# CEED/Laghos

Measured on AMD Instinct MI355X. Metric: Mdofs×steps/s on 3D Sedov -pa (Q3/Q2), higher is better.
Workload: dtype f64; 1 GPU; 3D Sedov -p 1 -m cube01_hex -rs 4 -ok 3 -ot 2 -pa (32^3 elements, E0/2^dim = 0.125); transport=none (one rank), elements=32768, h1_dofs=2738019, l2_dofs=884736, quad_points_per_element=216, rk_stages_executed=1300, ode=RK4, parallelism=elements1x1x1, zones_per_gpu=32x32x32

## Files before the change

include/laghos_hip.h:

```cpp
#ifndef LAGHOS_HIP_H
#define LAGHOS_HIP_H

#ifdef __cplusplus
extern "C" {
#endif

#define LGH_OK 0
#define LGH_ERR_ARG 1
#define LGH_ERR_UNSUPPORTED 2
#define LGH_ERR_HIP 3
#define LGH_ERR_COMM 4

#define LGH_SPACE_H1 0
#define LGH_SPACE_L2 1

typedef struct lgh_ctx lgh_ctx;

typedef struct lgh_config
{
   int dim, NE;
   int D1D, Q1D, L1D;
   int N;
   const int *h1_map;
   const double *B_h1;
// ... 20 lines not shown
void *lgh_stream(lgh_ctx *ctx);

double *lgh_qdata_stressJinvT(lgh_ctx *ctx);
double *lgh_qdata_Jac0inv(lgh_ctx *ctx);
double *lgh_qdata_rho0DetJ0w(lgh_ctx *ctx);
double *lgh_mass_D(lgh_ctx *ctx);
int lgh_mass_data_form(lgh_ctx *ctx, int *form);
int lgh_jac0inv_form(lgh_ctx *ctx, int *compact);
int lgh_mass_data_changed(lgh_ctx *ctx);
double *lgh_mass_diag(lgh_ctx *ctx);
int lgh_set_h0(lgh_ctx *ctx, double h0);
int lgh_get_h0(lgh_ctx *ctx, double *h0);
int lgh_set_dt_est(lgh_ctx *ctx, double dt_est);
int lgh_get_dt_est(lgh_ctx *ctx, double *dt_est);

int lgh_setup_rho0detj0(lgh_ctx *ctx, const double *x0, const double *rho0_l2,
                        const double *rho0_q, double *volume);

int lgh_force_mult(lgh_ctx *ctx, const double *x_l2, double *y_h1);
int lgh_force_mult_transpose(lgh_ctx *ctx, const double *v_h1, double *y_l2);

int lgh_mass_set_essential_tdofs(lgh_ctx *ctx, int comp);
int lgh_mass_eliminate_rhs(lgh_ctx *ctx, double *b);
int lgh_mass_mult(lgh_ctx *ctx, int space, const double *x, double *y);
int lgh_mass_mult_full(lgh_ctx *ctx, int space, const double *x, double *y);

int lgh_cg_solve(lgh_ctx *ctx, int space, const double *b, double *x, double rel_tol,
                 int max_iter, int *iters);
int lgh_l2_mass_solve_local(lgh_ctx *ctx, const double *b, double *x);

int lgh_qupdate(lgh_ctx *ctx, const double *S);
int lgh_qupdate_set_tiny_grad(lgh_ctx *ctx, double tiny_grad);
int lgh_qupdate_discard(lgh_ctx *ctx, int *mode, double *C_F);
int lgh_set_fused_forces(lgh_ctx *ctx, int on);
int lgh_qupdate_store_stress(lgh_ctx *ctx, int on);
int lgh_qupdate_stores_stress(lgh_ctx *ctx, int *on);
int lgh_qupdate_form(lgh_ctx *ctx, int *form);
int lgh_reset_quadrature_data(lgh_ctx *ctx);
int lgh_fused_force_mult(lgh_ctx *ctx, double *y_h1);
int lgh_fused_force_mult_transpose(lgh_ctx *ctx, double *y_l2);
int lgh_fused_force_e(lgh_ctx *ctx, double *y_e);
int lgh_quadrature_generation(lgh_ctx *ctx, unsigned long *gen, int *f1_valid, int *ftv_valid);
int lgh_get_fused_forces(lgh_ctx *ctx, int *f1, int *ftv);

int lgh_solve_velocity(lgh_ctx *ctx, const double *S, double *dS_dt, const double *one_l2,
                       double *rhs_h1, double *work_B, double rel_tol, int max_iter,
                       int *h1_iters);
int lgh_solve_energy(lgh_ctx *ctx, const double *S, const double *v_h1, double *dS_dt,
                     double *e_rhs, const double *e_source, double rel_tol, int max_iter,
                     int *l2_iters);
int lgh_solve_energy_begin(lgh_ctx *ctx, const double *S, const double *v_h1, double *dS_dt,
                           double *e_rhs, const double *e_source, double rel_tol, int max_iter);
int lgh_solve_energy_end(lgh_ctx *ctx, int *l2_iters);
int lgh_energy_lockstep_stats(lgh_ctx *ctx, long out[4]);

int lgh_vec_set(lgh_ctx *ctx, double *y, double a, long n);
int lgh_vec_copy(lgh_ctx *ctx, double *y, const double *x, long n);
int lgh_vec_axpby_pair(lgh_ctx *ctx, double *z1, double a1, const double *x1, double b1, double *z2, double a2, const double *x2, double b2,
                       const double *y, long n);
int lgh_vec_axpby(lgh_ctx *ctx, double *z, double a, const double *x, double b,
                  const double *y, long n);
int lgh_vec_dot(lgh_ctx *ctx, const double *x, const double *y, long n, double *result);
int lgh_vec_fingerprint(lgh_ctx *ctx, const double *x, long n, unsigned long long offset, unsigned long long out[2]);
int lgh_vec_fingerprint_shape(lgh_ctx *ctx, const double *x, long n, long out[4]);
int lgh_fingerprint_host(const void *words, long n, unsigned long long offset, unsigned long long out[2]);

// ... 106 lines not shown
```

laghos_amd/_lib.py:

```python
import ctypes
import os

_HERE = os.path.dirname(os.path.abspath(__file__))
LIB_PATH = os.path.join(_HERE, "liblaghos_hip.so")

c_dp = ctypes.c_void_p
c_int_p = ctypes.POINTER(ctypes.c_int)
c_dbl_p = ctypes.POINTER(ctypes.c_double)


class LghConfig(ctypes.Structure):
    _fields_ = [
        ("dim", ctypes.c_int), ("NE", ctypes.c_int),
        ("D1D", ctypes.c_int), ("Q1D", ctypes.c_int), ("L1D", ctypes.c_int),
        ("N", ctypes.c_int),
        ("h1_map", c_int_p),
        ("B_h1", c_dbl_p), ("G_h1", c_dbl_p), ("B_l2", c_dbl_p),
        ("weights", c_dbl_p), ("gamma", c_dbl_p),
        ("ess_count", ctypes.c_int * 3),
        ("ess", c_int_p * 3),
        ("owner", c_dbl_p),
        ("use_viscosity", ctypes.c_int), ("use_vorticity", ctypes.c_int),
        ("cfl", ctypes.c_double),
        ("order_v", ctypes.c_int),
# ... 49 lines not shown
    "lgh_vec_fingerprint_shape": (_I, [_P, _P, _L, ctypes.POINTER(ctypes.c_long)]),
    "lgh_fingerprint_host": (_I, [_P, _L, ctypes.c_ulonglong, ctypes.POINTER(ctypes.c_ulonglong)]),
    "lgh_internal_energy": (_I, [_P, _P, c_dbl_p]),
    "lgh_kinetic_energy": (_I, [_P, _P, c_dbl_p]),
    "lgh_sedov_setup": (_I, [_I, _D, _D, _D, _D, c_dbl_p]),
    "lgh_sedov_shock": (_I, [c_dbl_p, _D, c_dbl_p]),
    "lgh_sedov_eval_point": (_I, [c_dbl_p, _D, _D, c_dbl_p, c_dbl_p, c_dbl_p]),
    "lgh_sedov_eval": (_I, [_P, c_dbl_p, _D, _L, _P, _P, _P, _P]),
    "lgh_compute_density": (_I, [_P, _P, _P]),
    "lgh_sedov_density_error": (_I, [_P, _P, _P, c_dbl_p, _D, c_dbl_p, _I, c_dbl_p, c_dbl_p, c_dbl_p, c_dbl_p, c_dbl_p]),
    "lgh_sample_fields": (_I, [_P, _P, _P, _I, c_dbl_p, c_dbl_p, _P, _P, _P, _P, _P]),
    "lgh_sample_derived": (_I, [_P, _P, _I, c_dbl_p, c_dbl_p, c_dbl_p, _P, _P, _P, _P, _P]),
    "lgh_diagnostics_zones": (_I, [_P, _P, _P]),
    "lgh_diagnostics": (_I, [_P, _P, c_dbl_p]),
    "lgh_profile": (_I, [_P, _P, ctypes.POINTER(LghProfileSpec), c_dbl_p, ctypes.POINTER(ctypes.c_long)]),
    "lgh_get_timers": (_I, [_P, c_dbl_p, ctypes.POINTER(ctypes.c_long)]),
    "lgh_reset_timers": (_I, [_P]),
    "lgh_enable_timers": (_I, [_P, _I]),
    "lgh_ktime_begin": (_I, [_P, _I, _I]),
    "lgh_ktime_end": (_I, [_P, c_int_p, c_dbl_p]),
    "lgh_table_symmetry": (_I, [_P, c_int_p, c_int_p]),
    "lgh_k1_form": (_I, [_P, c_int_p]),
    "lgh_l2_mass_form": (_I, [_P, c_int_p, c_int_p]),
    "lgh_vcg_layout_stats": (_I, [_P, ctypes.POINTER(ctypes.c_long)]),
    "lgh_energy_lockstep_stats": (_I, [_P, ctypes.POINTER(ctypes.c_long)]),
    "lgh_mesh_order": (_I, [_P, ctypes.POINTER(ctypes.c_long)]),
    "lgh_mesh_order_host": (_I, [_I, _I, _I, _I, c_int_p, c_int_p, c_int_p, ctypes.POINTER(ctypes.c_long)]),
    "lgh_mass_data_form": (_I, [_P, c_int_p]),
    "lgh_jac0inv_form": (_I, [_P, c_int_p]),
    "lgh_mass_data_changed": (_I, [_P]),
    "lgh_comm_stats": (_I, [_P, c_int_p, ctypes.POINTER(ctypes.c_long), ctypes.POINTER(ctypes.c_long), c_int_p, c_int_p]),
    "lgh_qupdate_set_tiny_grad": (_I, [_P, _D]),
    "lgh_qupdate_discard": (_I, [_P, c_int_p, c_dbl_p]),
    "lgh_set_fused_forces": (_I, [_P, _I]),
    "lgh_qupdate_store_stress": (_I, [_P, _I]),
    "lgh_qupdate_stores_stress": (_I, [_P, c_int_p]),
    "lgh_qupdate_form": (_I, [_P, c_int_p]),
    "lgh_reset_quadrature_data": (_I, [_P]),
    "lgh_fused_force_mult": (_I, [_P, _P]),
    "lgh_fused_force_mult_transpose": (_I, [_P, _P]),
    "lgh_fused_force_e": (_I, [_P, _P]),
    "lgh_quadrature_generation": (_I, [_P, ctypes.POINTER(ctypes.c_ulong), c_int_p, c_int_p]),
    "lgh_get_fused_forces": (_I, [_P, c_int_p, c_int_p]),
    "lgh_comm_unique_id": (_I, [ctypes.c_char_p]),
    "lgh_comm_unique_id_shm": (_I, [ctypes.c_char_p]),
    "lgh_comm_init": (_I, [_P, _I, _I, ctypes.c_char_p]),
    "lgh_comm_set_neighbors": (_I, [_P, _I, c_int_p, c_int_p, ctypes.POINTER(c_int_p)]),
    "lgh_groups_to_neighbors": (_I, [_I, _I, _I, c_int_p, c_int_p, c_int_p, c_int_p, c_int_p, c_dbl_p, c_int_p, c_int_p,
                                     c_int_p, _I, c_int_p, _L]),
    "lgh_halo_sum": (_I, [_P, _P, _I]),
    "lgh_allreduce": (_I, [_P, c_dbl_p, _I]),
    "lgh_force_mult_E": (_I, [_P, _P, _P, _P]),
    "lgh_force_mult_transpose_E": (_I, [_P, _P, _P, _P]),
    "lgh_mass_apply_E": (_I, [_P, _I, _P, _P]),
    "lgh_test_vcg_k1": (_I, [_P, _P, _P, c_dbl_p, c_dbl_p, _I, _P, c_dbl_p]),
    "lgh_test_vcg_merged_faces": (_I, [_P, _P, ctypes.POINTER(ctypes.c_long)]),
    "lgh_test_vcg_k2": (_I, [_P, _I, _P, _P, _P, _P, c_dbl_p, c_dbl_p, c_dbl_p, c_dbl_p, c_dbl_p, ctypes.POINTER(ctypes.c_int)]),
    "lgh_test_exact_sum": (_I, [_P, _I, _L, _I, _I, c_dbl_p, c_dbl_p, ctypes.POINTER(ctypes.c_longlong),
                                ctypes.POINTER(ctypes.c_longlong), c_dbl_p, c_int_p]),
    "lgh_test_set_rank": (_I, [_P, _I, _I]),
    "lgh_test_word_peers": (_I, [_P, _I, ctypes.POINTER(ctypes.c_long)]),
    "lgh_test_halo_pack": (_I, [_P, _P, _I, _P]),
    "lgh_test_halo_combine": (_I, [_P, _P, _P, _I]),
    "lgh_test_rccl_self_sendrecv": (_I, [_P, _I, c_dbl_p]),
    "lgh_test_eig": (_I, [_P, _I, _I, _P, _P, _P]),
    "lgh_test_singular": (_I, [_P, _I, _I, _P, _P]),
# ... 38 lines not shown
```

laghos_amd/context.py:

```python
import ctypes

import numpy as np
import torch

from . import _lib
from ._lib import LghConfig, check


def _np_i32(a):
    return np.ascontiguousarray(a, dtype=np.int32)


def _np_f64(a):
    return np.ascontiguousarray(a, dtype=np.float64)


def _ptr(t):
    assert t.is_cuda and t.dtype == torch.float64 and t.is_contiguous()
    return ctypes.c_void_p(t.data_ptr())


def _dbl(a):
    assert isinstance(a, np.ndarray) and a.dtype == np.float64 and a.flags.c_contiguous
    return a.ctypes.data_as(_lib.c_dbl_p)
# ... 195 lines not shown

    def force_mult_transpose(self, v_h1, y_l2):
        check(self.lib.lgh_force_mult_transpose(self.h, _ptr(v_h1), _ptr(y_l2)))

    def mass_set_ess(self, comp):
        check(self.lib.lgh_mass_set_essential_tdofs(self.h, comp))

    def mass_eliminate_rhs(self, b):
        check(self.lib.lgh_mass_eliminate_rhs(self.h, _ptr(b)))

    def mass_mult(self, space, x, y, full=False):
        fn = self.lib.lgh_mass_mult_full if full else self.lib.lgh_mass_mult
        check(fn(self.h, space, _ptr(x), _ptr(y)))

    def cg_solve(self, space, b, x, rel_tol, max_iter):
        it = ctypes.c_int(0)
        check(self.lib.lgh_cg_solve(self.h, space, _ptr(b), _ptr(x), rel_tol, max_iter, ctypes.byref(it)))
        return it.value

    def l2_mass_solve_local(self, b, x):
        check(self.lib.lgh_l2_mass_solve_local(self.h, _ptr(b), _ptr(x)))

    def qupdate(self, S):
        check(self.lib.lgh_qupdate(self.h, _ptr(S)))

    def qupdate_set_tiny_grad(self, v):
        check(self.lib.lgh_qupdate_set_tiny_grad(self.h, float(v)))

    def qupdate_discard(self):
        m, cf = ctypes.c_int(-1), ctypes.c_double(0.0)
        check(self.lib.lgh_qupdate_discard(self.h, ctypes.byref(m), ctypes.byref(cf)))
        return m.value, cf.value

    def table_symmetry(self):
        a, b = ctypes.c_int(-1), ctypes.c_int(-1)
        check(self.lib.lgh_table_symmetry(self.h, ctypes.byref(a), ctypes.byref(b)))
        return a.value, b.value

    def k1_form(self):
        f = ctypes.c_int(-2)
        check(self.lib.lgh_k1_form(self.h, ctypes.byref(f)))
        return {0: "column", 2: "plane", 4: "slab", 5: "kron"}.get(f.value)

    def mesh_order(self):
        o = (ctypes.c_long * 8)()
        check(self.lib.lgh_mesh_order(self.h, o))
        return dict(structured=bool(o[0]), identity=bool(o[1]), components=int(o[2]), extent=(int(o[3]), int(o[4]), int(o[5])))

    def test_vcg_k1(self, r, d_old, rz, rz_prev, first):
        y = self.empty(3 * self.NE * self.ND)
        rz, rzp, den = _np_f64(rz), _np_f64(rz_prev), np.zeros(3)
        check(self.lib.lgh_test_vcg_k1(self.h, _ptr(r), _ptr(d_old) if d_old is not None else None, _dbl(rz), _dbl(rzp),
                                       int(bool(first)), _ptr(y), _dbl(den)))
        return y.view(3, -1), den

    def test_vcg_merged_faces(self):
        mask = np.zeros(self.NE * self.ND, dtype=np.uint8)
        n = ctypes.c_long(0)
        check(self.lib.lgh_test_vcg_merged_faces(self.h, mask.ctypes.data_as(ctypes.c_void_p), ctypes.byref(n)))
        return mask, n.value

    def test_vcg_k2(self, it, y_E, r, d, x, den, rz, rz_prev, alpha_prev):
        den, rz, rzp, al, out = _np_f64(den), _np_f64(rz), _np_f64(rz_prev), _np_f64(alpha_prev), np.zeros(3)
        form = ctypes.c_int(-1)
        check(self.lib.lgh_test_vcg_k2(self.h, int(it), _ptr(y_E), _ptr(r), _ptr(d), _ptr(x), _dbl(den), _dbl(rz), _dbl(rzp),
                                       _dbl(al), _dbl(out), ctypes.byref(form)))
# ... 264 lines not shown
```

laghos_amd/csrc/lgh_api.hip:

```cpp
#include <cstdarg>
#include <cstdlib>
#include <cmath>
#include <algorithm>
#include <limits>

#include "lgh_common.hpp"

#include <atomic>
#include <chrono>
#include <dlfcn.h>

namespace lgh
{

static thread_local char g_err[512] = "";
void set_error(const char *fmt, ...)
{
   va_list ap;
   va_start(ap, fmt);
   vsnprintf(g_err, sizeof(g_err), fmt, ap);
   va_end(ap);
}

__global__ void __launch_bounds__(256) vec_set_k(double *y, double a, long n)
// ... 245 lines not shown
   s.slab_exact = env_flag("LGH_SLAB_EXACT", 1);
   s.slab_merge = env_flag("LGH_SLAB_MERGE", 1);
   s.slab_defer = env_flag("LGH_SLAB_DEFER", 1);
   s.slab_ye_wide = env_flag("LGH_SLAB_YE_WIDE", 0);
   s.slab_dyn = env_flag("LGH_SLAB_DYN", -1);
   s.rz_limbs = env_flag("LGH_RZ_LIMBS", 1);
   s.kron_neb = env_flag("LGH_KRON_NEB", 1);
   s.fused_init = env_flag("LGH_FUSED_INIT", 1);
   s.k2p = env_flag("LGH_K2P", 1);
   s.k2_skip = env_flag("LGH_K2_SKIP", 1);
   s.k2_grid = (int)env_long("LGH_K2_GRID", 0);
   s.k2_node_weight = env_long("LGH_K2_NODE_WEIGHT", 5);
   s.order = env_flag("LGH_ORDER", 1);
   s.order_multi = env_flag("LGH_ORDER_MULTI", 1);
   s.comm2 = env_flag("LGH_COMM2", -1);
   s.force_multi = env_flag("LGH_FORCE_MULTI", 0);
   s.halo_piggyback = env_flag("LGH_HALO_PIGGYBACK", 1);
   s.halo_fused_pack = env_flag("LGH_HALO_FUSED_PACK", 1);
   s.overlap = env_flag("LGH_OVERLAP", 1);
   s.energy_lockstep = env_flag("LGH_ENERGY_LOCKSTEP", 1);
   s.spin = env_flag("LGH_SPIN", 1);
   s.mass_sep = env_flag("LGH_MASS_SEP", 1);
   s.mass_kron = env_flag("LGH_MASS_KRON", 1);
   s.mass_rank1 = env_flag("LGH_MASS_RANK1", 1);
   s.mass_rank1_tol = env_double("LGH_MASS_RANK1_TOL", kMassRank1Tol);
   s.l2_neb = env_flag("LGH_L2_NEB", 1);
   s.l2_plane = env_flag("LGH_L2_PLANE", 1);
   s.l2_fused = env_flag("LGH_L2_FUSED", 1);
   s.q_form = env_flag("LGH_Q_FORM", 1);
   s.q_ppt = env_flag("LGH_Q_PPT", 0);
   s.q_swz = (int)env_long("LGH_Q_SWZ", -1);
   s.q_occ4 = env_flag("LGH_Q_OCC4", -1);
   s.q_discard = (int)env_long("LGH_Q_DISCARD", 1);
   s.q_tiny_grad = env_double("LGH_Q_TINY_GRAD", 1e-30);
   s.fused_ftv = env_flag("LGH_FUSED_FTV", 1);
   s.fused_f1 = env_flag("LGH_FUSED_F1", 1);
   s.b_sym = env_flag("LGH_B_SYM", 1);
   s.jac0_compact = env_flag("LGH_JAC0_COMPACT", 1);
   s.jac0_tol = std::min(std::max(env_double("LGH_JAC0_TOL", kJac0Tol), 0.0), 1e-10);
   s.profile_fold = (int)std::max(0L, env_long("LGH_PROFILE_FOLD", 8));
   s.roctx = env_flag("LGH_ROCTX", 0);
   s.vcg_trace = env_string("LGH_VCG_TRACE");
   s.vcg_trace_phases = getenv("LGH_VCG_TRACE_PHASES") != nullptr;
   s.q_trace = env_string("LGH_Q_TRACE");
   s.q_trace_call = (int)env_long("LGH_Q_TRACE_CALL", 40);
   return s;
}

template <typename T> static int dev_alloc_copy(T **dst, const T *src, size_t n)
{
   LGH_HIP_CHECK(hipMalloc((void **)dst, std::max<size_t>(n, 1) * sizeof(T)));
   if (src && n) { LGH_HIP_CHECK(hipMemcpy(*dst, src, n * sizeof(T), hipMemcpyHostToDevice)); }
   return LGH_OK;
}
template <typename T> static int dev_alloc_zero(T **dst, size_t n)
{
   LGH_HIP_CHECK(hipMalloc((void **)dst, std::max<size_t>(n, 1) * sizeof(T)));
   LGH_HIP_CHECK(hipMemset(*dst, 0, std::max<size_t>(n, 1) * sizeof(T)));
   LGH_HIP_CHECK(hipStreamSynchronize(nullptr));
   return LGH_OK;
}

static bool kernel_id_supported(int id)
{
   switch (id)
   {
// ... 181 lines not shown
      {
         ok = std::fabs(w1[i] - w1[Q - 1 - i]) <= 8.9e-16 * w1[i];
         w1[Q - 1 - i] = w1[i];
      }
      for (int q = 0; ok && q < c->NQ; q++)
      {
         const int qx = q % Q, qy = (q / Q) % Q, qz = q / (Q * Q);
         const double prod = (dim == 3) ? w1[qx] * w1[qy] * w1[qz] : w1[qx] * w1[qy];
         ok = std::fabs(prod - cfg->weights[q]) <= 1.8e-15 * std::fabs(cfg->weights[q]);
      }
      if (ok && c->sw.mass_sep) { LGH_TRY(dev_alloc_copy(&c->w1d, w1.data(), (size_t)Q)); }
      if (c->w1d && c->sw.mass_kron)
      {
         auto tile = [&](const double *Bt, const int n, double **out) -> int {
            std::vector<double> M((size_t)n * n);
            for (int i = 0; i < n; i++)
            {
               for (int j = 0; j < n; j++)
               {
                  long double s = 0.0L;
                  for (int q = 0; q < Q; q++) { s += (long double)Bt[q + Q * i] * (long double)w1[q] * (long double)Bt[q + Q * j]; }
                  M[(size_t)i + (size_t)n * j] = (double)s;
               }
            }
            return dev_alloc_copy(out, M.data(), M.size());
         };
         LGH_TRY(tile(cfg->B_h1, c->D1D, &c->M1h));
         LGH_TRY(tile(cfg->B_l2, c->L1D, &c->M1l));
      }
   }
   LGH_TRY(dev_alloc_copy(&c->gamma, cfg->gamma, (size_t)c->NE));
   const size_t nmap = (size_t)c->NE * c->ND;
   LGH_TRY(dev_alloc_copy(&c->h1map, cfg->h1_map, nmap));
   LGH_TRY(mesh_order_build(c, cfg->h1_map));
   {
      std::vector<int> off((size_t)c->N + 1, 0), idx(nmap);
      for (size_t i = 0; i < nmap; i++)
      {
         const int n = cfg->h1_map[i];
         if (n < 0 || n >= c->N) { set_error("h1_map entry out of range"); return LGH_ERR_ARG; }
         off[(size_t)n + 1]++;
      }
      for (int n = 0; n < c->N; n++) { off[(size_t)n + 1] += off[n]; }
      std::vector<int> pos(off.begin(), off.end() - 1);
      for (size_t i = 0; i < nmap; i++) { idx[pos[cfg->h1_map[i]]++] = (int)i; }
      LGH_TRY(dev_alloc_copy(&c->t_off, off.data(), off.size()));
      LGH_TRY(dev_alloc_copy(&c->t_idx, idx.data(), idx.size()));
      int deg = 0;
      for (int n = 0; n < c->N; n++) { deg = std::max(deg, off[(size_t)n + 1] - off[n]); }
      std::vector<int> ell((size_t)deg * c->N, -1);
      for (int n = 0; n < c->N; n++)
         for (int k = off[n]; k < off[(size_t)n + 1]; k++) { ell[(size_t)(k - off[n]) * c->N + n] = idx[k]; }
      c->t_deg = deg;
      LGH_TRY(dev_alloc_copy(&c->t_ell, ell.data(), ell.size()));
   }
   for (int k = 0; k < 3; k++)
   {
      c->ess_count[k] = (k < dim) ? cfg->ess_count[k] : 0;
      std::vector<uint8_t> mask((size_t)c->N, 0);
      for (int i = 0; i < c->ess_count[k]; i++)
      {
         const int n = cfg->ess[k][i];
         if (n < 0 || n >= c->N) { set_error("essential dof out of range"); return LGH_ERR_ARG; }
         mask[n] = 1;
      }
      LGH_TRY(dev_alloc_copy(&c->essmask[k], mask.data(), mask.size()));
// ... 95 lines not shown
void *lgh_stream(lgh_ctx *c) { return c ? (void *)c->stream : nullptr; }

static void invalidate_fused(lgh_ctx *c)
{
   c->fused_ftv_valid = 0;
   c->fused_f1_valid = 0;
   c->qgen++;
}
double *lgh_qdata_stressJinvT(lgh_ctx *c)
{
   invalidate_fused(c);
   if (c->stress_store) { c->stress_current = 1; }
   return c->stressJinvT;
}
static int no_1d(const lgh_ctx *c, const char *who)
{
   if (c->dim != 1) { return LGH_OK; }
   set_error("%s: not available for a 1D context (lgh_1d.hip has its own kernels)", who);
   return LGH_ERR_UNSUPPORTED;
}
int lgh_qupdate_form(lgh_ctx *c, int *form)
{
   LGH_CHECK_ARG(c && form);
   *form = qupdate_form(c);
   return LGH_OK;
}
int lgh_qupdate_discard(lgh_ctx *c, int *mode, double *C_F)
{
   LGH_CHECK_ARG(c && mode && C_F);
   *mode = c->q_discard;
   *C_F = c->q_cF;
   return LGH_OK;
}
int lgh_qupdate_stores_stress(lgh_ctx *c, int *on)
{
   LGH_CHECK_ARG(c && on);
   *on = (!c->stress_store && c->erhs_q && c->force_e_q && c->v_snap && !c->fused_forces_off && c->dim == 3) ? 0 : 1;
   return LGH_OK;
}
int lgh_qupdate_store_stress(lgh_ctx *c, int on)
{
   LGH_CHECK_ARG(c);
   if ((on != 0) != (c->stress_store != 0))
   {
      c->stress_store = on ? 1 : 0;
      invalidate_fused(c);
      c->stress_current = 0;
   }
   return LGH_OK;
}
int lgh_reset_quadrature_data(lgh_ctx *c)
{
   LGH_CHECK_ARG(c);
   invalidate_fused(c);
   return LGH_OK;
}
int lgh_fused_force_mult(lgh_ctx *c, double *y_h1)
{
   LGH_CHECK_ARG(c && y_h1);
   if (!(c->force_e_q && c->fused_f1_valid)) { set_error("lgh_fused_force_mult: no fused F.1 on hand"); return LGH_ERR_ARG; }
   int rc = h1_transpose_gather(c, c->dim, c->force_e_q, y_h1);
   if (rc == LGH_OK && c->multi != 0) { rc = halo_sum(c, y_h1, c->dim); }
   return rc;
}
int lgh_fused_force_e(lgh_ctx *c, double *y_e)
{
// ... 577 lines not shown
```

laghos_amd/csrc/lgh_common.hpp:

```cpp
#pragma once
#include <hip/hip_runtime.h>

#include <algorithm>
#include <cstdint>
#include <cstdio>
#include <cstring>
#include <string>
#include <vector>

#include "../../include/laghos_hip.h"

namespace lgh
{

void set_error(const char *fmt, ...);

#define LGH_HIP_CHECK(expr)                                                              \
   do                                                                                    \
   {                                                                                     \
      hipError_t e_ = (expr);                                                            \
      if (e_ != hipSuccess)                                                              \
      {                                                                                  \
         lgh::set_error("HIP error %s at %s:%d: %s", hipGetErrorName(e_), __FILE__,      \
                        __LINE__, #expr);                                                \
// ... 54 lines not shown
constexpr int kPinResult = 0;
constexpr int kPinDot = 1;
constexpr int kPinReduceOut = 2, kPinReduceIn = 3;
constexpr int kPinDt = 8, kPinDtFlag = 9, kPinDtToken = 10;
constexpr int kPinVcg = 32;
constexpr int kPinVcgToken = 80;
static_assert(sizeof(CgScalars) <= kPinDt * sizeof(double) && kPinDtFlag == kPinDt + 1 && kPinDtToken == kPinDt + 2 && kPinDtToken < kPinVcg &&
              kPinVcgToken < kPinDoubles, "slots of the pinned block: disjoint, inside the allocation");

struct Timers
{
   bool enabled = true;
   hipEvent_t ev[2] = {nullptr, nullptr};
   double t[4] = {0, 0, 0, 0};
   long c[3] = {0, 0, 0};
};

struct KTime
{
   int which = -1, max = 0, n = 0;
   std::vector<hipEvent_t> ev;
};

struct Comm;

struct MeshOrder
{
   bool structured = false, identity = true;
   int components = 0, extent[3] = {0, 0, 0};
   std::vector<int> zorder;
   std::vector<int> nnum;
   std::vector<int> ncaller;
   int *zorder_d = nullptr, *ncaller_d = nullptr, *nnum_d = nullptr;
};

constexpr double kMassRank1Tol = 1e-12;
constexpr double kJac0Tol = 1e-12;

struct Switches
{
   int vcg_variant;
   int slab_wide, slab_exact, slab_merge, slab_defer, slab_ye_wide;
   int slab_dyn;
   int rz_limbs, kron_neb, fused_init;
   int k2p, k2_skip, k2_grid;
   long k2_node_weight;
   int order, order_multi;
   int comm2;
   int force_multi, halo_piggyback, halo_fused_pack, overlap, energy_lockstep, spin;
   int mass_sep, mass_kron, mass_rank1, l2_neb, l2_plane, l2_fused;
   double mass_rank1_tol;
   int q_form, q_ppt, q_swz, fused_ftv, fused_f1, b_sym, jac0_compact;
   int q_occ4;
   int q_discard;
   double q_tiny_grad;
   double jac0_tol;
   int profile_fold;
   int roctx, vcg_trace_phases, q_trace_call;
   std::string vcg_trace, q_trace;
};
Switches read_switches();

struct ScalarCg;

struct EnergySolve
{
   enum Mode
   {
      Idle,
      Overlapped,
      Deferred,
      Lockstep
   };
   Mode mode = Idle;
   bool polled = false;
   int iters = 0;
   struct { const double *S, *v; double *dS, *e_rhs; const double *src; double tol; int maxit; } args = {};
};

}

struct lgh_ctx
{
   lgh::Switches sw;
   int dim, NE, D1D, Q1D, L1D, ND, NQ, NL, N, H1V, L2V;
   int kid;
   bool visc, vort;
   double cfl, h0, h1order;
   double q_tiny_grad;
   int q_discard;
   double q_cF;
   int device;
   hipStream_t stream;
   hipStream_t stream2;
   int on_stream2;
   hipEvent_t ev_fork, ev_join;
   lgh::ScalarCg *l2run = nullptr;
   const double *accel_src;
   lgh::EnergySolve energy;
   long ls_stats[3] = {0, 0, 0};
   bool own_stream;

   double *B, *G, *Bl, *W, *gamma;
   int *h1map;
   int *t_off;
   int *t_idx;
   int *t_ell;
   int t_deg;
   uint8_t *essmask[3];
   int *ess[3];
   int ess_count[3];
   double *owner;
   int cur_ess;

   double *stressJinvT, *Jac0inv, *rho0DetJ0w, *massD, *diagV, *dinvV;
   double *Jac0inv_soa;
   double *Jac0inv_e;
   int jac0_compact;
   double *massS, *ones_ne;
   double *M1h = nullptr, *M1l = nullptr;
   double *w1d = nullptr;
   int mass_rank1;
   double *dt_est_dev;
   double *erhs_q;
   double *v_snap;
   double *force_e_q;
   int fused_ftv_valid, fused_f1_valid;
   unsigned long qgen;
   int *dev_flags;
   double *ones_l2;
   int stress_store;
   int stress_current;
   int fused_forces_off;
   double *XE;
   double *YE;
   double *cg_r, *cg_z, *cg_d0, *cg_d1, *cg_y;
   double *partials;
// ... 380 lines not shown
```

laghos_amd/csrc/lgh_order.hip:

```cpp
#include "lgh_common.hpp"

#include <algorithm>
#include <array>
#include <cstdlib>
#include <numeric>

namespace lgh
{

static void free_order(MeshOrder *o)
{
   if (!o) { return; }
   (void)hipFree(o->zorder_d);
   (void)hipFree(o->ncaller_d);
   (void)hipFree(o->nnum_d);
   delete o;
}
void mesh_order_free(lgh_ctx *c)
{
   free_order((MeshOrder *)c->order);
   c->order = nullptr;
}

static bool analyse(const int *map, const int NE, const int N, const int D, MeshOrder &o)
// ... 95 lines not shown
   std::iota(o.zorder.begin(), o.zorder.end(), 0);
   auto zkey = [&](const int e) {
      const int cc = comp[e];
      return std::array<long, 4>{cc, ijk[e][2] - cmin[cc][2], ijk[e][1] - cmin[cc][1], ijk[e][0] - cmin[cc][0]};
   };
   std::sort(o.zorder.begin(), o.zorder.end(), [&](const int x, const int y) { return zkey(x) < zkey(y); });
   std::vector<std::array<long, 4>> nkey((size_t)N, std::array<long, 4>{-1, 0, 0, 0});
   for (int i = 0; i < NE; i++)
   {
      const int e = o.zorder[i];
      const auto zk = zkey(e);
      for (int d = 0; d < ND; d++)
      {
         const int n = map[(size_t)e * ND + d];
         if (nkey[n][0] >= 0) { continue; }
         const int dx = d % D, dy = (d / D) % D, dz = d / (D * D);
         nkey[n] = {zk[0], zk[1] * p + dz, zk[2] * p + dy, zk[3] * p + dx};
      }
   }
   o.ncaller.resize((size_t)N);
   std::iota(o.ncaller.begin(), o.ncaller.end(), 0);
   auto nk = [&](const int n) { return nkey[n][0] >= 0 ? nkey[n] : std::array<long, 4>{(long)ncomp, 0, 0, (long)n}; };
   std::sort(o.ncaller.begin(), o.ncaller.end(), [&](const int x, const int y) {
      const auto kx = nk(x), ky = nk(y);
      return kx < ky || (kx == ky && x < y);
   });
   o.nnum.resize((size_t)N);
   for (int m = 0; m < N; m++) { o.nnum[o.ncaller[m]] = m; }
   o.components = ncomp;
   for (int b = 0; b < 3; b++) { o.extent[b] = cmax[0][b] - cmin[0][b] + 1; }
   return true;
}

int mesh_order_build(lgh_ctx *c, const int *map)
{
   mesh_order_free(c);
   MeshOrder *o = new MeshOrder();
   c->order = o;
   if (c->dim != 3 || !c->sw.order) { return LGH_OK; }
   o->structured = analyse(map, c->NE, c->N, c->D1D, *o);
   if (!o->structured)
   {
      o->zorder.clear();
      o->nnum.clear();
      o->ncaller.clear();
      return LGH_OK;
   }
   bool ident = true;
   for (int e = 0; ident && e < c->NE; e++) { ident = o->zorder[e] == e; }
   for (int n = 0; ident && n < c->N; n++) { ident = o->ncaller[n] == n; }
   o->identity = ident;
   if (ident) { return LGH_OK; }
   LGH_HIP_CHECK(hipMalloc((void **)&o->zorder_d, (size_t)c->NE * sizeof(int)));
   LGH_HIP_CHECK(hipMalloc((void **)&o->ncaller_d, (size_t)c->N * sizeof(int)));
   LGH_HIP_CHECK(hipMalloc((void **)&o->nnum_d, (size_t)c->N * sizeof(int)));
   LGH_HIP_CHECK(hipMemcpy(o->zorder_d, o->zorder.data(), (size_t)c->NE * sizeof(int), hipMemcpyHostToDevice));
   LGH_HIP_CHECK(hipMemcpy(o->ncaller_d, o->ncaller.data(), (size_t)c->N * sizeof(int), hipMemcpyHostToDevice));
   LGH_HIP_CHECK(hipMemcpy(o->nnum_d, o->nnum.data(), (size_t)c->N * sizeof(int), hipMemcpyHostToDevice));
   return LGH_OK;
}

__global__ void __launch_bounds__(256) order_gather_k(const double *__restrict__ in, const int *__restrict__ idx, double *__restrict__ out, const int N, const int ncomp)
{
   const int m = blockIdx.x * blockDim.x + threadIdx.x;
   if (m >= N) { return; }
   const int n = idx[m];
   for (int c = 0; c < ncomp; c++) { out[(size_t)c * N + m] = in[(size_t)c * N + n]; }
}
__global__ void __launch_bounds__(256) order_scatter_k(const double *__restrict__ in, const int *__restrict__ idx, double *__restrict__ out, const int N, const int ncomp)
{
   const int m = blockIdx.x * blockDim.x + threadIdx.x;
   if (m >= N) { return; }
   const int n = idx[m];
   for (int c = 0; c < ncomp; c++) { out[(size_t)c * N + n] = in[(size_t)c * N + m]; }
}
__global__ void __launch_bounds__(256) order_gather_u8_k(const uint8_t *__restrict__ in, const int *__restrict__ idx, uint8_t *__restrict__ out, const int N)
{
   const int m = blockIdx.x * blockDim.x + threadIdx.x;
   if (m < N) { out[m] = in[idx[m]]; }
}
__global__ void __launch_bounds__(256) order_blocks_k(const double *__restrict__ in, const int *__restrict__ idx, double *__restrict__ out, const size_t nblk, const int per,
                                                      const int scatter)
{
   const size_t t = (size_t)blockIdx.x * blockDim.x + threadIdx.x;
   if (t >= nblk * per) { return; }
   const size_t i = t / per, k = t - i * per;
   const size_t j = (size_t)idx[i];
   if (scatter) { out[j * per + k] = in[t]; }
   else { out[t] = in[j * per + k]; }
}

// ... 21 lines not shown
int order_zone_blocks(lgh_ctx *c, const double *in, double *out, int per, bool to_caller)
{
   const MeshOrder *o = (const MeshOrder *)c->order;
   const size_t n = (size_t)c->NE * per;
   hipLaunchKernelGGL(order_blocks_k, dim3((unsigned)((n + 255) / 256)), dim3(256), 0, c->stream, in, o->zorder_d, out, (size_t)c->NE, per, to_caller ? 1 : 0);
   LGH_HIP_CHECK(hipGetLastError());
   return LGH_OK;
}

}

extern "C" int lgh_mesh_order_host(int dim, int NE, int N, int D1D, const int *h1_map, int *zorder, int *nnum, long out[8])
{
   LGH_CHECK_ARG(h1_map && zorder && nnum && out && NE > 0 && N > 0 && D1D >= 2);
   for (int i = 0; i < 8; i++) { out[i] = 0; }
   for (int e = 0; e < NE; e++) { zorder[e] = e; }
   for (int n = 0; n < N; n++) { nnum[n] = n; }
   out[1] = 1;
   if (dim != 3) { return LGH_OK; }
   const size_t nmap = (size_t)NE * D1D * D1D * D1D;
   for (size_t i = 0; i < nmap; i++) { LGH_CHECK_ARG(h1_map[i] >= 0 && h1_map[i] < N); }
   lgh::MeshOrder o;
   if (!lgh::analyse(h1_map, NE, N, D1D, o)) { return LGH_OK; }
   bool ident = true;
   for (int e = 0; e < NE; e++) { zorder[e] = o.zorder[e]; ident = ident && o.zorder[e] == e; }
   for (int n = 0; n < N; n++) { nnum[n] = o.nnum[n]; ident = ident && o.nnum[n] == n; }
   out[0] = 1;
   out[1] = ident ? 1 : 0;
   out[2] = o.components;
   for (int b = 0; b < 3; b++) { out[3 + b] = o.extent[b]; }
   return LGH_OK;
}

extern "C" int lgh_mesh_order(lgh_ctx *c, long out[8])
{
   LGH_CHECK_ARG(c && out);
   const lgh::MeshOrder *o = (const lgh::MeshOrder *)c->order;
   for (int i = 0; i < 8; i++) { out[i] = 0; }
   if (!o) { return LGH_OK; }
   out[0] = o->structured ? 1 : 0;
   out[1] = o->identity ? 1 : 0;
   out[2] = o->components;
   out[3] = o->extent[0];
   out[4] = o->extent[1];
   out[5] = o->extent[2];
   return LGH_OK;
}
```

laghos_amd/csrc/lgh_qpoint.hpp:

```cpp
#pragma once
#include "lgh_common.hpp"
#include "lgh_smallmat.hpp"

namespace lgh
{

enum { QMODE_UPDATE = 0, QMODE_SETUP = 1, QMODE_IE = 2, QMODE_KE = 3 };

struct QArgs
{
   int NE, N;
   const double *B, *G, *Bl, *W;
   const int *map;
   const double *x, *v, *e;
   const double *gamma;
   const double *rho0DetJ0w_in;
   const double *Jac0inv_in;
   const double *Jac0inv_soa;
   const double *Jac0inv_e;
   double *Jac0inv_soa_out;
   double *stressJinvT;
   double *Jac0inv_out, *rho0DetJ0w_out, *massD_out;
   const double *rho0_q;
   double *partials;
   unsigned int *ticket;
   double *result;
   double h0, h1order, cfl;
   int visc, vort;
   double *force_e;
   double *erhs_q;
   int q_swz;
   const int *zorder;
   double tiny_grad;
   int discard;
   double f1_quiet;
};

__device__ __forceinline__ double smooth_step_01(double x, double eps)
{
   const double y = (x + eps) / (2.0 * eps);
   if (y < 0.0) { return 0.0; }
   if (y > 1.0) { return 1.0; }
   return (3.0 - 2.0 * y) * y * y;
}

template <int DIM, bool VISC = true>
__device__ __forceinline__ double qpoint_body(const QArgs &a, const int e, const size_t eq,
                                              const double weight, const double *J, const double *dV,
                                              const double e_val, const size_t plane,
                                              const double *J0i, const double rho0DetJ0w, double &ftv, double *sjw,
                                              const double dt_ref, bool *dt_skipped = nullptr)
{
   constexpr int DIM2 = DIM * DIM;
   double Jinv[DIM2], stress[DIM2], sgrad_v[DIM2], stressJiT[DIM2];
   const double gamma = a.gamma[e];
   const double inv_weight = 1. / weight;
   const double detJ = sm::det<DIM>(J);
   sm::inverse<DIM>(J, detJ, Jinv);
   const double R = inv_weight * rho0DetJ0w / detJ;
   const double E = fmax(0.0, e_val);
   const double P = (gamma - 1.0) * R * E;
   const double S = sm::fsqrt(gamma * (gamma - 1.0) * E);
#pragma unroll
   for (int k = 0; k < DIM2; k++) { stress[k] = 0.0; }
#pragma unroll
// ... 732 lines not shown

static QArgs q_base(lgh_ctx *c)
{
   QArgs a;
   memset(&a, 0, sizeof(a));
   a.NE = c->NE;
   a.N = c->N;
   a.B = c->B;
   a.G = c->G;
   a.Bl = c->Bl;
   a.W = c->W;
   a.map = c->h1map;
   a.gamma = c->gamma;
   a.rho0DetJ0w_in = c->rho0DetJ0w;
   a.Jac0inv_in = c->Jac0inv;
   a.Jac0inv_soa = c->Jac0inv_soa;
   a.stressJinvT = c->stressJinvT;
   a.partials = c->partials + 2 * (size_t)c->part_stride;
   a.ticket = c->tickets + 2 * kTicketSlot;
   a.h0 = c->h0;
   a.h1order = c->h1order;
   a.cfl = c->cfl;
   a.visc = c->visc;
   a.vort = c->vort;
   a.tiny_grad = c->q_tiny_grad;
   a.discard = c->q_discard;
   a.f1_quiet = (c->q_cF > 0.0) ? (2.220446049250313e-16 * 2.220446049250313e-16) / (2.0 * c->q_cF) : 0.0;
   a.q_swz = c->sw.q_swz;
   a.erhs_q = c->fused_forces_off ? nullptr : c->erhs_q;
   a.force_e = (c->dim == 3 && !c->fused_forces_off) ? c->force_e_q : nullptr;
   {
      const MeshOrder *o = mesh_order(c);
      a.zorder = o ? o->zorder_d : nullptr;
   }
   return a;
}

}
```

laghos_amd/csrc/lgh_qrows.hpp:

```cpp
#pragma once
#include "lgh_qpoint.hpp"

namespace lgh
{

template <int D, int Q, int L> struct QRows
{
   static constexpr int ND = D * D * D, NQ = Q * Q * Q, NL = L * L * L, NF = 6;
   static constexpr int SU = NF * ND;
   static constexpr int SX = NF * Q * D * D;
   static constexpr int SFS = 9 * NQ + NQ;
   static constexpr int R1 = (SU + 2 * SX > SFS) ? SU + 2 * SX : SFS;
   static constexpr int SY = 3 * NF * Q * Q * D;
   static constexpr int SE = NL + L * L * Q + L * Q * Q;
   static constexpr int ST = 2 * Q * D + Q * L;
   static constexpr int TOTAL = R1 + SY + SE + ST;
};

template <int NIN, int NOUT>
__device__ __forceinline__ void row_fwd(const double *__restrict__ T, const double (&in)[NIN], double (&out)[NOUT])
{
#pragma unroll
   for (int q = 0; q < NOUT; q++)
   {
      double s = T[q * NIN] * in[0];
#pragma unroll
      for (int d = 1; d < NIN; d++) { s = fma(T[q * NIN + d], in[d], s); }
      out[q] = s;
   }
}
template <int NIN, int NOUT>
__device__ __forceinline__ void row_bwd(const double *__restrict__ T, const double (&in)[NIN], double (&out)[NOUT])
{
#pragma unroll
// ... 17 lines not shown
qrows_kernel(const QArgs a, unsigned long long *trace = nullptr)
{
   unsigned long long tstamp[12];
#define LGH_QSTAMP(K_) do { if (TRACE) { tstamp[K_] = wall_clock64(); } } while (0)
   LGH_QSTAMP(0);
   using S = QRows<D, Q, L>;
   constexpr int ND = S::ND, NQ = S::NQ, NL = S::NL, NF = S::NF, NT = NQ;
   constexpr int DD = D * D, QQ = Q * Q;
   __shared__ __attribute__((aligned(16))) double smem[S::TOTAL];
   double *const sR1 = smem;
   double *const sU = sR1;
   double *const sX = sR1 + S::SU;
   double *const sF = sR1;
   double *const sS = sR1 + 9 * NQ;
   double *const sW = sR1;
   double *const sY = smem + S::R1;
   double *const sA = sY;
   double *const sTB = sY + S::SY;
   double *const sTG = sTB + Q * D;
   double *const sTL = sTG + Q * D;
   double *const sE = sTL + Q * L;
   double *const sE1 = sE + NL;
   double *const sE2 = sE1 + L * L * Q;

   const int lt = threadIdx.x;
   const int tx = lt % Q, ty = (lt / Q) % Q, tz = lt / QQ;
   int e = blockIdx.x;
   if (a.q_swz < 0) { e = xcd_swizzle(blockIdx.x, gridDim.x); }
   else if (a.q_swz > 0)
   {
      const int R = 1 << a.q_swz, span = 8 * R, b = blockIdx.x;
      if (b < (int)(gridDim.x / span) * span) { e = (b / span) * span + (b & 7) * R + ((b >> 3) & (R - 1)); }
   }
   if (a.zorder) { e = __builtin_amdgcn_readfirstlane(a.zorder[min(e, a.NE - 1)]); }
   const size_t eq = (size_t)e * NQ + lt;
   const size_t plane = (size_t)a.NE * NQ;

   for (int i = lt; i < Q * D; i += NT)
   {
      const int q = i / D, d = i - q * D;
      sTB[i] = a.B[q + Q * d];
      sTG[i] = a.G[q + Q * d];
   }
   for (int i = lt; i < Q * L; i += NT)
   {
      const int q = i / L, l = i - q * L;
      sTL[i] = a.Bl[q + Q * l];
   }
   for (int i = lt; i < 3 * ND; i += NT)
   {
      const int c = i / ND, d = i - c * ND;
      const size_t n = (size_t)c * a.N + a.map[(size_t)e * ND + d];
      sU[i] = a.x[n];
      sU[i + 3 * ND] = a.v[n];
   }
   for (int i = lt; i < NL; i += NT) { sE[i] = a.e[(size_t)e * NL + i]; }
   double J0i[9];
   if (J0C)
   {
#pragma unroll
      for (int k = 0; k < 9; k++) { J0i[k] = uniform_f64(a.Jac0inv_e[(size_t)9 * e + k]); }
   }
   else
   {
#pragma unroll
      for (int k = 0; k < 9; k++) { J0i[k] = a.Jac0inv_soa[eq + plane * k]; }
   }
   const double rdw = a.rho0DetJ0w_in[eq];
   const double weight = a.W[lt];
   const bool hint_on = a.visc && (a.discard & kQDiscardDt);
   double dt_ref = __builtin_inf();
   if (hint_on)
   {
      dt_ref = uniform_f64(__longlong_as_double((long long)__hip_atomic_load((const unsigned long long *)(a.result + kDtHint), __ATOMIC_RELAXED,
                                                                            __HIP_MEMORY_SCOPE_AGENT)));
   }
   LGH_QSTAMP(1);
   __syncthreads();
   LGH_QSTAMP(2);

   for (int i = lt; i < 2 * NF * DD; i += NT)
   {
      const int which = i / (NF * DD), r = i - which * (NF * DD);
      const double *T = sTB + which * (Q * D);
      double u[D], o[Q];
      row_load<D>(sU + D * r, u);
      row_fwd<D, Q>(T, u, o);
      const int f = r / DD, zy = r - f * DD;
      double *dst = sX + which * S::SX + f * (Q * DD) + zy;
#pragma unroll
      for (int q = 0; q < Q; q++) { dst[q * DD] = o[q]; }
   }
   {
      const int j = NT - 1 - lt;
      if (j < L * L)
      {
         double u[L], o[Q];
         row_load<L>(sE + L * j, u);
         row_fwd<L, Q>(sTL, u, o);
#pragma unroll
         for (int q = 0; q < Q; q++) { sE1[j * Q + q] = o[q]; }
      }
   }
   __syncthreads();
   LGH_QSTAMP(3);

   for (int i = lt; i < 3 * NF * Q * D; i += NT)
   {
      const int part = i / (NF * Q * D), r = i - part * (NF * Q * D);
      const double *T = sTB + ((part == 1) ? Q * D : 0);
// ... 298 lines not shown
```

Baseline: 1730 Mdofs*steps/s.

## Hoist qupdate prologue loads into registers and compute structured H1 map indices

The quadrature-update kernel prologue now issues all its global loads into registers first and writes them to shared memory afterwards. This exposes more memory-level parallelism instead of serialized load-store loops. It also removes the dependent zorder→map→x/v indirection, either with a precomputed z-ordered copy of the map or, when the mesh is structured, by computing node indices arithmetically with magic-number division. The cost is more registers and extra host setup, and the arithmetic path relies on detecting a regular map layout.

After: 1725 Mdofs*steps/s. About the same (-0.3%).

```diff
diff --git a/include/laghos_hip.h b/include/laghos_hip.h
--- a/include/laghos_hip.h
+++ b/include/laghos_hip.h
@@ -76,6 +76,8 @@
 int lgh_qupdate(lgh_ctx *ctx, const double *S);
 int lgh_qupdate_set_tiny_grad(lgh_ctx *ctx, double tiny_grad);
 int lgh_qupdate_discard(lgh_ctx *ctx, int *mode, double *C_F);
+int lgh_map_formula(lgh_ctx *ctx, int *ok);
+int lgh_map_formula_host(int dim, int NE, int N, int D1D, const int *h1_map, long out[10]);
 int lgh_set_fused_forces(lgh_ctx *ctx, int on);
 int lgh_qupdate_store_stress(lgh_ctx *ctx, int on);
 int lgh_qupdate_stores_stress(lgh_ctx *ctx, int *on);
diff --git a/laghos_amd/_lib.py b/laghos_amd/_lib.py
--- a/laghos_amd/_lib.py
+++ b/laghos_amd/_lib.py
@@ -105,6 +105,8 @@
     "lgh_comm_stats": (_I, [_P, c_int_p, ctypes.POINTER(ctypes.c_long), ctypes.POINTER(ctypes.c_long), c_int_p, c_int_p]),
     "lgh_qupdate_set_tiny_grad": (_I, [_P, _D]),
     "lgh_qupdate_discard": (_I, [_P, c_int_p, c_dbl_p]),
+    "lgh_map_formula": (_I, [_P, c_int_p]),
+    "lgh_map_formula_host": (_I, [_I, _I, _I, _I, c_int_p, ctypes.POINTER(ctypes.c_long)]),
     "lgh_set_fused_forces": (_I, [_P, _I]),
     "lgh_qupdate_store_stress": (_I, [_P, _I]),
     "lgh_qupdate_stores_stress": (_I, [_P, c_int_p]),
diff --git a/laghos_amd/context.py b/laghos_amd/context.py
--- a/laghos_amd/context.py
+++ b/laghos_amd/context.py
@@ -251,6 +251,11 @@
         check(self.lib.lgh_qupdate_discard(self.h, ctypes.byref(m), ctypes.byref(cf)))
         return m.value, cf.value
 
+    def map_formula(self):
+        ok = ctypes.c_int(-1)
+        check(self.lib.lgh_map_formula(self.h, ctypes.byref(ok)))
+        return ok.value
+
     def table_symmetry(self):
         a, b = ctypes.c_int(-1), ctypes.c_int(-1)
         check(self.lib.lgh_table_symmetry(self.h, ctypes.byref(a), ctypes.byref(b)))
diff --git a/laghos_amd/csrc/lgh_api.hip b/laghos_amd/csrc/lgh_api.hip
--- a/laghos_amd/csrc/lgh_api.hip
+++ b/laghos_amd/csrc/lgh_api.hip
@@ -301,6 +301,7 @@
    s.q_swz = (int)env_long("LGH_Q_SWZ", -1);
    s.q_occ4 = env_flag("LGH_Q_OCC4", -1);
    s.q_discard = (int)env_long("LGH_Q_DISCARD", 1);
+   s.q_mapf = env_flag("LGH_Q_MAPF", 1);
    s.q_tiny_grad = env_double("LGH_Q_TINY_GRAD", 1e-30);
    s.fused_ftv = env_flag("LGH_FUSED_FTV", 1);
    s.fused_f1 = env_flag("LGH_FUSED_F1", 1);
@@ -548,6 +549,7 @@
    LGH_TRY(dev_alloc_copy(&c->gamma, cfg->gamma, (size_t)c->NE));
    const size_t nmap = (size_t)c->NE * c->ND;
    LGH_TRY(dev_alloc_copy(&c->h1map, cfg->h1_map, nmap));
+   if (c->sw.q_mapf) { c->smap = find_map_formula(cfg->h1_map, dim, c->NE, c->N, c->D1D); }
    LGH_TRY(mesh_order_build(c, cfg->h1_map));
    {
       std::vector<int> off((size_t)c->N + 1, 0), idx(nmap);
@@ -709,6 +711,13 @@
    *C_F = c->q_cF;
    return LGH_OK;
 }
+int lgh_map_formula(lgh_ctx *c, int *ok)
+{
+   LGH_CHECK_ARG(c && ok);
+   const MeshOrder *o = mesh_order(c);
+   *ok = (o && o->zmap_d) ? 2 : (c->smap.ok && !o) ? 1 : 0;
+   return LGH_OK;
+}
 int lgh_qupdate_stores_stress(lgh_ctx *c, int *on)
 {
    LGH_CHECK_ARG(c && on);
diff --git a/laghos_amd/csrc/lgh_common.hpp b/laghos_amd/csrc/lgh_common.hpp
--- a/laghos_amd/csrc/lgh_common.hpp
+++ b/laghos_amd/csrc/lgh_common.hpp
@@ -110,7 +110,17 @@
    std::vector<int> nnum;
    std::vector<int> ncaller;
    int *zorder_d = nullptr, *ncaller_d = nullptr, *nnum_d = nullptr;
-};
+   DevPtr<int> zmap_d;
+};
+
+struct StructuredMap
+{
+   int ok;
+   int nex, ney;
+   int b0, Ex, Ey, Ez, sx, sy, sz;
+   unsigned long long mx, my;
+};
+StructuredMap find_map_formula(const int *map, int dim, int NE, int N, int D);
 
 constexpr double kMassRank1Tol = 1e-12;
 constexpr double kJac0Tol = 1e-12;
@@ -131,6 +141,7 @@
    int q_form, q_ppt, q_swz, fused_ftv, fused_f1, b_sym, jac0_compact;
    int q_occ4;
    int q_discard;
+   int q_mapf;
    double q_tiny_grad;
    double jac0_tol;
    int profile_fold;
@@ -181,6 +192,7 @@
 
    double *B, *G, *Bl, *W, *gamma;
    int *h1map;
+   lgh::StructuredMap smap;
    int *t_off;
    int *t_idx;
    int *t_ell;
diff --git a/laghos_amd/csrc/lgh_order.hip b/laghos_amd/csrc/lgh_order.hip
--- a/laghos_amd/csrc/lgh_order.hip
+++ b/laghos_amd/csrc/lgh_order.hip
@@ -151,6 +151,44 @@
    return true;
 }
 
+StructuredMap find_map_formula(const int *map, const int dim, const int NE, const int N, const int D)
+{
+   StructuredMap m;
+   memset(&m, 0, sizeof(m));
+   if (dim != 3 || D < 2 || NE < 1 || !map) { return m; }
+   const int ND = D * D * D;
+   auto base = [&](const long e) { return (long)map[(size_t)e * ND]; };
+   const long sx = (long)map[1] - map[0], sy = (long)map[D] - map[0], sz = (long)map[D * D] - map[0];
+   const long Ex = (NE > 1) ? base(1) - base(0) : 0;
+   long nex = 1;
+   while (nex < NE && base(nex) - base(nex - 1) == Ex) { nex++; }
+   const long Ey = (nex < NE) ? base(nex) - base(0) : 0;
+   long ney = 1;
+   while (ney * nex < NE && base(ney * nex) - base((ney - 1) * nex) == Ey) { ney++; }
+   const long Ez = (nex * ney < NE) ? base(nex * ney) - base(0) : 0;
+   if (base(0) < 0 || sx < 0 || sy < 0 || sz < 0 || Ex < 0 || Ey < 0 || Ez < 0) { return m; }
+   const unsigned long long mx = (1ull << 32) / (unsigned long long)nex + 1, my = (1ull << 32) / (unsigned long long)ney + 1;
+   for (long e = 0; e < NE; e++)
+   {
+      const long t = e / nex, ex = e - t * nex, ez = t / ney, ey = t - ez * ney;
+      if ((long)(((unsigned long long)e * mx) >> 32) != t || (long)(((unsigned long long)t * my) >> 32) != ez) { return m; }
+      const long b = base(0) + ex * Ex + ey * Ey + ez * Ez;
+      const int *me = map + (size_t)e * ND;
+      for (int d = 0; d < ND; d++)
+      {
+         const int dx = d % D, dy = (d / D) % D, dz = d / (D * D);
+         const long n = b + dx * sx + dy * sy + dz * sz;
+         if (n >= (long)N || (long)me[d] != n) { return m; }
+      }
+   }
+   m.nex = (int)nex; m.ney = (int)ney;
+   m.b0 = (int)base(0); m.Ex = (int)Ex; m.Ey = (int)Ey; m.Ez = (int)Ez;
+   m.sx = (int)sx; m.sy = (int)sy; m.sz = (int)sz;
+   m.mx = mx; m.my = my;
+   m.ok = 1;
+   return m;
+}
+
 int mesh_order_build(lgh_ctx *c, const int *map)
 {
    mesh_order_free(c);
@@ -176,6 +214,14 @@
    LGH_HIP_CHECK(hipMemcpy(o->zorder_d, o->zorder.data(), (size_t)c->NE * sizeof(int), hipMemcpyHostToDevice));
    LGH_HIP_CHECK(hipMemcpy(o->ncaller_d, o->ncaller.data(), (size_t)c->N * sizeof(int), hipMemcpyHostToDevice));
    LGH_HIP_CHECK(hipMemcpy(o->nnum_d, o->nnum.data(), (size_t)c->N * sizeof(int), hipMemcpyHostToDevice));
+   if (c->sw.q_mapf)
+   {
+      const size_t ND = (size_t)c->ND;
+      std::vector<int> zmap((size_t)c->NE * ND);
+      for (size_t i = 0; i < (size_t)c->NE; i++) { std::copy_n(map + (size_t)o->zorder[i] * ND, ND, zmap.begin() + i * ND); }
+      int rc = o->zmap_d.upload(zmap.data(), zmap.size());
+      if (rc) { return rc; }
+   }
    return LGH_OK;
 }
 
@@ -263,6 +309,15 @@
    return LGH_OK;
 }
 
+extern "C" int lgh_map_formula_host(int dim, int NE, int N, int D1D, const int *h1_map, long out[10])
+{
+   LGH_CHECK_ARG(h1_map && out && NE > 0 && N > 0 && D1D >= 2);
+   const lgh::StructuredMap m = lgh::find_map_formula(h1_map, dim, NE, N, D1D);
+   const long v[10] = {m.ok, m.nex, m.ney, m.b0, m.Ex, m.Ey, m.Ez, m.sx, m.sy, m.sz};
+   for (int i = 0; i < 10; i++) { out[i] = v[i]; }
+   return LGH_OK;
+}
+
 extern "C" int lgh_mesh_order(lgh_ctx *c, long out[8])
 {
    LGH_CHECK_ARG(c && out);
diff --git a/laghos_amd/csrc/lgh_qpoint.hpp b/laghos_amd/csrc/lgh_qpoint.hpp
--- a/laghos_amd/csrc/lgh_qpoint.hpp
+++ b/laghos_amd/csrc/lgh_qpoint.hpp
@@ -31,6 +31,8 @@
    double *erhs_q;
    int q_swz;
    const int *zorder;
+   const int *zmap;
+   StructuredMap smap;
    double tiny_grad;
    int discard;
    double f1_quiet;
@@ -829,6 +831,8 @@
    {
       const MeshOrder *o = mesh_order(c);
       a.zorder = o ? o->zorder_d : nullptr;
+      a.zmap = o ? o->zmap_d.p : nullptr;
+      if (!o) { a.smap = c->smap; }
    }
    return a;
 }
diff --git a/laghos_amd/csrc/lgh_qrows.hpp b/laghos_amd/csrc/lgh_qrows.hpp
--- a/laghos_amd/csrc/lgh_qrows.hpp
+++ b/laghos_amd/csrc/lgh_qrows.hpp
@@ -1,5 +1,7 @@
 #pragma once
 #include "lgh_qpoint.hpp"
+
+#include <type_traits>
 
 namespace lgh
 {
@@ -83,50 +85,125 @@
       const int R = 1 << a.q_swz, span = 8 * R, b = blockIdx.x;
       if (b < (int)(gridDim.x / span) * span) { e = (b / span) * span + (b & 7) * R + ((b >> 3) & (R - 1)); }
    }
-   if (a.zorder) { e = __builtin_amdgcn_readfirstlane(a.zorder[min(e, a.NE - 1)]); }
+   static_assert(Q * D <= NT && Q * L <= NT && NL <= NT, "one pass per table and for the L2 field");
+   constexpr int NGI = (3 * ND + NT - 1) / NT;
+   double gx[NGI], gv[NGI], tb_, tg_, tl_, ge, weight, rdw, J0i[9];
+   unsigned long long hint_raw;
+   const bool hint_on = a.visc && (a.discard & kQDiscardDt);
+   auto p0_loads = [&](auto gm_) {
+      constexpr int GM = decltype(gm_)::value;
+      const int zi = min(e, a.NE - 1);
+      int zraw, gn[NGI];
+      if (GM != 1 && a.zorder) { zraw = a.zorder[zi]; }
+      if (GM == 2)
+      {
+#pragma unroll
+         for (int k = 0; k < NGI; k++)
+         {
+            const int i = lt + k * NT;
+            if (i < 3 * ND) { gn[k] = a.zmap[(size_t)zi * ND + (i % ND)]; }
+         }
+      }
+      if (GM == 1)
+      {
+         const int t = (int)(((unsigned long long)(unsigned)e * a.smap.mx) >> 32), ex = e - t * a.smap.nex;
+         const int ez = (int)(((unsigned long long)(unsigned)t * a.smap.my) >> 32), ey = t - ez * a.smap.ney;
+         const int base = a.smap.b0 + ex * a.smap.Ex + ey * a.smap.Ey + ez * a.smap.Ez;
+#pragma unroll
+         for (int k = 0; k < NGI; k++)
+         {
+            const int i = lt + k * NT;
+            if (i < 3 * ND)
+            {
+               const int c = i / ND, d = i - c * ND, dx = d % D, dy = (d / D) % D, dz = d / DD;
+               const size_t n = (size_t)c * a.N + (size_t)(base + dx * a.smap.sx + dy * a.smap.sy + dz * a.smap.sz);
+               gx[k] = a.x[n];
+               gv[k] = a.v[n];
+            }
+         }
+      }
+      if (lt < Q * D)
+      {
+         const int q = lt / D, d = lt - q * D;
+         tb_ = a.B[q + Q * d];
+         tg_ = a.G[q + Q * d];
+      }
+      if (lt < Q * L)
+      {
+         const int q = lt / L, l = lt - q * L;
+         tl_ = a.Bl[q + Q * l];
+      }
+      weight = a.W[lt];
+      if (hint_on) { hint_raw = __hip_atomic_load((const unsigned long long *)(a.result + kDtHint), __ATOMIC_RELAXED, __HIP_MEMORY_SCOPE_AGENT); }
+      if (GM != 1 && a.zorder) { e = __builtin_amdgcn_readfirstlane(zraw); }
+      if (GM == 0)
+      {
+#pragma unroll
+         for (int k = 0; k < NGI; k++)
+         {
+            const int i = lt + k * NT;
+            if (i < 3 * ND) { gn[k] = a.map[(size_t)e * ND + (i % ND)]; }
+         }
+      }
+      if (lt < NL) { ge = a.e[(size_t)e * NL + lt]; }
+      const size_t eq_ = (size_t)e * NQ + lt, plane_ = (size_t)a.NE * NQ;
+      if (J0C)
+      {
+#pragma unroll
+         for (int k = 0; k < 9; k++) { J0i[k] = a.Jac0inv_e[(size_t)9 * e + k]; }
+         rdw = a.rho0DetJ0w_in[eq_];
+      }
+      if (GM != 1)
+      {
+#pragma unroll
+         for (int k = 0; k < NGI; k++)
+         {
+            const int i = lt + k * NT;
+            if (i < 3 * ND)
+            {
+               const size_t n = (size_t)(i / ND) * a.N + gn[k];
+               gx[k] = a.x[n];
+               gv[k] = a.v[n];
+            }
+         }
+      }
+   };
+   if (a.zmap) { p0_loads(std::integral_constant<int, 2>()); }
+   else if (a.smap.ok) { p0_loads(std::integral_constant<int, 1>()); }
+   else { p0_loads(std::integral_constant<int, 0>()); }
    const size_t eq = (size_t)e * NQ + lt;
    const size_t plane = (size_t)a.NE * NQ;
-
-   for (int i = lt; i < Q * D; i += NT)
-   {
-      const int q = i / D, d = i - q * D;
-      sTB[i] = a.B[q + Q * d];
-      sTG[i] = a.G[q + Q * d];
-   }
-   for (int i = lt; i < Q * L; i += NT)
-   {
-      const int q = i / L, l = i - q * L;
-      sTL[i] = a.Bl[q + Q * l];
-   }
-   for (int i = lt; i < 3 * ND; i += NT)
-   {
-      const int c = i / ND, d = i - c * ND;
-      const size_t n = (size_t)c * a.N + a.map[(size_t)e * ND + d];
-      sU[i] = a.x[n];
-      sU[i + 3 * ND] = a.v[n];
-   }
-   for (int i = lt; i < NL; i += NT) { sE[i] = a.e[(size_t)e * NL + i]; }
-   double J0i[9];
+   if (!J0C)
+   {
+#pragma unroll
+      for (int k = 0; k < 9; k++) { J0i[k] = a.Jac0inv_soa[eq + plane * k]; }
+      rdw = a.rho0DetJ0w_in[eq];
+   }
+   LGH_QSTAMP(1);
    if (J0C)
    {
 #pragma unroll
-      for (int k = 0; k < 9; k++) { J0i[k] = uniform_f64(a.Jac0inv_e[(size_t)9 * e + k]); }
-   }
-   else
-   {
-#pragma unroll
-      for (int k = 0; k < 9; k++) { J0i[k] = a.Jac0inv_soa[eq + plane * k]; }
-   }
-   const double rdw = a.rho0DetJ0w_in[eq];
-   const double weight = a.W[lt];
-   const bool hint_on = a.visc && (a.discard & kQDiscardDt);
+      for (int k = 0; k < 9; k++) { J0i[k] = uniform_f64(J0i[k]); }
+   }
    double dt_ref = __builtin_inf();
-   if (hint_on)
-   {
-      dt_ref = uniform_f64(__longlong_as_double((long long)__hip_atomic_load((const unsigned long long *)(a.result + kDtHint), __ATOMIC_RELAXED,
-                                                                            __HIP_MEMORY_SCOPE_AGENT)));
-   }
-   LGH_QSTAMP(1);
+   if (hint_on) { dt_ref = uniform_f64(__longlong_as_double((long long)hint_raw)); }
+   if (lt < Q * D)
+   {
+      sTB[lt] = tb_;
+      sTG[lt] = tg_;
+   }
+   if (lt < Q * L) { sTL[lt] = tl_; }
+#pragma unroll
+   for (int k = 0; k < NGI; k++)
+   {
+      const int i = lt + k * NT;
+      if (i < 3 * ND)
+      {
+         sU[i] = gx[k];
+         sU[i + 3 * ND] = gv[k];
+      }
+   }
+   if (lt < NL) { sE[lt] = ge; }
    __syncthreads();
    LGH_QSTAMP(2);
 
```
